# omnirevolve/omnirevolve-image-processor

Hardware: AMD Instinct MI355X
Metric: Mpx/s end-to-end (color->order) (higher is better)
Workload: dtype u8/i32 raster + f32/f64 geometry; 1 GPU; 4096x4096 BGR image, 8 colour layers, stages 02->12 (k-means fit, masks, edges, contours, scale, sort, intra dedup, cross dedup, plot order), default A4 canvas 8400x11880; parallelism=one GPU, one pipeline per colour layer, ops_last_step_rank0=4261, exchange=none

## Files before the change

### omnirevolve-image-processor_amd/csrc/vector08a.hip

```cpp
#include "vec08.h"
#include <rocprim/rocprim.hpp>
#include <type_traits>
#include <vector>

namespace {

template <class Src>
__global__ __launch_bounds__(128) void k_split_small08(Src src, int64_t n_polys, orip_params08 P, const PolyFeat* __restrict__ feat,
                                                        unsigned* __restrict__ is_tap, unsigned* __restrict__ is_keep, int2* __restrict__ tap_xy, GatherDesc* __restrict__ kd) {
    int64_t i = (int64_t)blockIdx.x * blockDim.x + threadIdx.x;
    if (i > n_polys) return;
    if (i == n_polys) { is_tap[i] = 0; is_keep[i] = 0; return; }
    const int64_t n = src.len(i);
    unsigned tap = 0, keep = 0;
    GatherDesc g; g.begin = src.off[i]; g.len = n; g.rev = 0; g.src = (int32_t)i;
    if (n >= 2) {
        const int32_t x0 = feat[i].x0, x1 = feat[i].x1, y0 = feat[i].y0, y1 = feat[i].y1;
        double d = (double)max(x1 - x0, y1 - y0);
        if (d <= P.tap_diam && d <= P.tap_max_dim && n <= (int64_t)P.tap_max_v) {
            double per; float cx, cy, r;
            if constexpr (std::is_same<Src, ESrc>::value) {
                const int32_t* p = reinterpret_cast<const int32_t*>(src.pts + src.off[i]);
                per = (double)vs::pairwise_seglen_sum<0>(p, n);
                if (per <= P.tap_max_per) vs::min_enclosing_circle(p, n, cx, cy, r);
// ... 272 lines not shown
    unsigned i = ord[r]; RsInfo ri = info[i];
    int64_t k = 0;
    if (!ri.pass) k = sample_seg(cum + off[i], ri.n_eff, (double)sample_t(g - sbase[r], step), -1, ri.n_eff - 2);
    hints[b] = make_int2((int)r, (int)k);
}
__device__ __forceinline__ unsigned smp_slot8(unsigned s) { return s ^ ((s >> 5) & 3u); }
__device__ __forceinline__ unsigned smp_slot4(unsigned s) { return s ^ ((s >> 6) & 3u); }
template <int CTRL, int ROWMASK>
__device__ __forceinline__ void wave_seg_step(double& a, unsigned& f) {
    const int lo = __builtin_amdgcn_update_dpp(0, __double2loint(a), CTRL, ROWMASK, 0xf, false);
    const int hi = __builtin_amdgcn_update_dpp(0, __double2hiint(a), CTRL, ROWMASK, 0xf, false);
    const unsigned pf = (unsigned)__builtin_amdgcn_update_dpp(0, (int)f, CTRL, ROWMASK, 0xf, false);
    if (!f) a = __dadd_rn(__hiloint2double(hi, lo), a);
    f |= pf;
}
template <class Src>
__global__ __launch_bounds__(256) void k_samples(Src src, const int64_t* __restrict__ cumoff, const float* __restrict__ cum,
                                                  const RsInfo* __restrict__ info, const unsigned* __restrict__ ord, const unsigned* __restrict__ sbase, int64_t n_rank,
                                                  unsigned MS, double step, int W, int H, SampleArrs A,
                                                  const int2* __restrict__ hints, unsigned nhb, unsigned long long* __restrict__ pixbits, int Wq, unsigned* __restrict__ firstseq) {
    constexpr int S = 4;
    constexpr unsigned NS = 256 * S;
    static_assert(NS == ORIP_SMP_BLOCK, "k_tail_par takes a block of k_samples for 1024 samples");
    __shared__ double shx[NS], shy[NS], shp[2], swa[4];
    __shared__ unsigned swf[4];
    __shared__ unsigned shr[NS];
    const unsigned g0 = (blockIdx.x * 256 + threadIdx.x) * S;
    if (g0 < MS) {
        const unsigned hb = g0 >> 8;
        const int2 h0 = hints[hb];
        const bool last = hb + 1 == nhb;
        const int2 h1 = last ? make_int2((int)n_rank - 1, 0) : hints[hb + 1];
        int64_t r = sample_rank(sbase, info, ord, h0.x + 1, (int64_t)h1.x + 1, g0);
        unsigned i = ord[r]; unsigned j = g0 - sbase[r];
        auto cu = src.cur(i); const float* s = cum + cumoff[i];
        RsInfo ri = info[i];
        int64_t kprev = -2;
        const unsigned j0 = j;
        auto pos_at = [&](int64_t k, double t, double& ox, double& oy) {
            double sk = (double)s[k], sk1 = (double)s[k + 1];
            double u = __ddiv_rn(__dsub_rn(t, sk), fmax(1e-6, __dsub_rn(sk1, sk)));
            double a = __dsub_rn(1.0, u);
            const int2 p0 = cu.at(k), p1 = cu.at(k + 1);
            ox = __dadd_rn(__dmul_rn((double)(float)p0.x, a), __dmul_rn((double)(float)p1.x, u));
            oy = __dadd_rn(__dmul_rn((double)(float)p0.y, a), __dmul_rn((double)(float)p1.y, u));
        };
#pragma unroll 1
        for (int u = 0; u < S; u++) {
            const unsigned g = g0 + (unsigned)u;
            if (g >= MS) break;
            if (u > 0 && j >= ri.m) {
                do { r++; i = ord[r]; ri = info[i]; } while (ri.m == 0);
                j = 0; cu = src.cur(i); s = cum + cumoff[i]; kprev = -2;
            }
            double x, y;
            if (ri.pass) { const int2 q = cu.at(j); x = (double)(float)q.x; y = (double)(float)q.y; }
            else {
                const double t = (double)sample_t(j, step);
                int64_t k;
                if (kprev < -1) {
                    const bool first = u == 0;
                    k = sample_seg(s, ri.n_eff, t, (first && r == h0.x) ? h0.y : -1, (first && !last && r == h1.x) ? h1.y : ri.n_eff - 2);
                } else {
                    k = kprev < 0 ? 0 : kprev;
                    const int64_t kmax = ri.n_eff - 2;
                    while (k < kmax) {
                        float v[8];
#pragma unroll
                        for (int q = 0; q < 8; q++) v[q] = (k + 1 + q <= kmax + 1) ? s[k + 1 + q] : __int_as_float(0x7f800000);
                        int cnt = 0; bool run = true;
#pragma unroll
                        for (int q = 0; q < 8; q++) { run = run && ((double)v[q] <= t); cnt += run ? 1 : 0; }
                        k += cnt;
                        if (cnt < 8) break;
                    }
                    if (k > kmax) k = kmax;
                }
                kprev = k;
                pos_at(k, t, x, y);
            }
            const unsigned ls = threadIdx.x * S + (unsigned)u;
            shx[smp_slot8(ls)] = x; shy[smp_slot8(ls)] = y;
            shr[smp_slot4(ls)] = (unsigned)r | (j == 0 ? 0x80000000u : 0u);
            j++;
        }
        if (j0 > 0 && threadIdx.x == 0) {
            int64_t r2 = sample_rank(sbase, info, ord, h0.x + 1, (int64_t)h1.x + 1, g0);
            const unsigned i2 = ord[r2]; cu = src.cur(i2); s = cum + cumoff[i2]; ri = info[i2];
            double qx, qy;
            if (ri.pass) { const int2 q = cu.at(j0 - 1); qx = (double)(float)q.x; qy = (double)(float)q.y; }
            else { const double t = (double)sample_t(j0 - 1, step); pos_at(sample_seg(s, ri.n_eff, t, -1, ri.n_eff - 2), t, qx, qy); }
            shp[0] = qx; shp[1] = qy;
        }
    }
    __syncthreads();
    const unsigned b0 = blockIdx.x * NS;
    double dd[S] = {0.0, 0.0, 0.0, 0.0};
#pragma unroll
    for (int u = 0; u < S; u++) {
        const unsigned ls = threadIdx.x + 256u * (unsigned)u, g = b0 + ls;
        if (g >= MS) break;
        const unsigned at = smp_slot8(ls);
        const double x = shx[at], y = shy[at];
        const unsigned rw = shr[smp_slot4(ls)];
        double d = 0.0;
        if (!(rw >> 31)) { const unsigned before = smp_slot8(ls ? ls - 1u : 0u); d = vs::norm2_f64(x - (ls ? shx[before] : shp[0]), y - (ls ? shy[before] : shp[1])); }
        A.dprev[g] = d; dd[u] = d;
        A.sx[g] = x; A.sy[g] = y; A.rank[g] = rw & 0x7fffffffu;
        const long long xi = vs::round_half_even(x), yi = vs::round_half_even(y);
        const bool in = xi >= 0 && yi >= 0 && xi < W && yi < H;
        A.pxy[g] = in ? ((unsigned)xi | ((unsigned)yi << 16) | ((rw >> 31) ? ORIP_PXY_FIRST : 0u)) : ORIP_PXY_OUT;
        if (pixbits && in) {
            unsigned long long* wp = &pixbits[(size_t)yi * Wq + (xi >> 6)]; const unsigned long long bit = 1ULL << (xi & 63);
            if (!(*wp & bit) && !(atomicOr(wp, bit) & bit)) firstseq[(size_t)yi * W + xi] = 0xffffffffu;
        }
    }
    __syncthreads();
#pragma unroll
    for (int u = 0; u < S; u++) shx[smp_slot8(threadIdx.x + 256u * (unsigned)u)] = dd[u];
    __syncthreads();
    const unsigned l0 = threadIdx.x * S;
    double v[S]; unsigned f[S];
#pragma unroll
    for (int q = 0; q < S; q++) { v[q] = shx[smp_slot8(l0 + q)]; f[q] = (b0 + l0 + q < MS) ? shr[smp_slot4(l0 + q)] >> 31 : 0u; }
    double wa = v[0]; unsigned wf = f[0];
#pragma unroll
    for (int q = 1; q < S; q++) { wa = f[q] ? v[q] : __dadd_rn(wa, v[q]); wf |= f[q]; }
    wave_seg_step<0x111, 0xf>(wa, wf); wave_seg_step<0x112, 0xf>(wa, wf); wave_seg_step<0x114, 0xf>(wa, wf); wave_seg_step<0x118, 0xf>(wa, wf);
    wave_seg_step<0x142, 0xa>(wa, wf); wave_seg_step<0x143, 0xc>(wa, wf);
    const int lane = threadIdx.x & 63, wv = threadIdx.x >> 6;
    if (lane == 63) { swa[wv] = wa; swf[wv] = wf; }
    double ea = __hiloint2double(__builtin_amdgcn_update_dpp(0, __double2hiint(wa), 0x138 , 0xf, 0xf, false),
                                 __builtin_amdgcn_update_dpp(0, __double2loint(wa), 0x138, 0xf, 0xf, false));
    const unsigned ef = (unsigned)__builtin_amdgcn_update_dpp(0, (int)wf, 0x138, 0xf, 0xf, false);
    __syncthreads();
    if (!ef) {
        double ca = 0.0;
        for (int k = 0; k < wv; k++) ca = swf[k] ? swa[k] : __dadd_rn(ca, swa[k]);
        ea = __dadd_rn(ca, ea);
    }
#pragma unroll
    for (int q = 0; q < S; q++) { ea = f[q] ? v[q] : __dadd_rn(ea, v[q]); v[q] = ea; }
    const unsigned gs = b0 + l0;
    if (gs + S <= MS) { double2* o = reinterpret_cast<double2*>(A.Sloc + gs); o[0] = make_double2(v[0], v[1]); o[1] = make_double2(v[2], v[3]); }
    else { for (int q = 0; q < S; q++) if (gs + q < MS) A.Sloc[gs + q] = v[q]; }
}

__device__ __forceinline__ double dpp_shr1_f64(double v) {
    const int lo = __builtin_amdgcn_update_dpp(0, __double2loint(v), 0x138 , 0xf, 0xf, true);
    const int hi = __builtin_amdgcn_update_dpp(0, __double2hiint(v), 0x138, 0xf, 0xf, true);
    return __hiloint2double(hi, lo);
}
__global__ __launch_bounds__(64) void k_tail_replay(const unsigned* __restrict__ sbase, int64_t n_rank, double T, SampleArrs A, unsigned* __restrict__ npop, const unsigned* __restrict__ only) {
    constexpr unsigned C = 1024u, RM = 2u * C - 1u;
    __shared__ double ops[64], rr[64];
    __shared__ double Dl[2 * C];
    __shared__ unsigned NPl[C];
    const int lane = threadIdx.x;
    for (int64_t r = blockIdx.x; r < n_rank; r += gridDim.x) {
        if (only && !only[r]) continue;
        const unsigned b = sbase[r], e = sbase[r + 1];
        if (e <= b) continue;
        const double* D = A.dprev + b; unsigned* NP = npop + b;
        const unsigned m = e - b;
        unsigned head = 0; double racc = 0.0;
        unsigned j0 = 0, cb = 0;
        auto fill = [&](unsigned c0) {
            double td[16]; unsigned tn[16];
#pragma unroll
            for (int u = 0; u < 16; u++) { const unsigned idx = c0 + (unsigned)lane + 64u * u; td[u] = D[idx < m ? idx : m - 1u]; tn[u] = NP[idx < m ? idx : m - 1u]; }
#pragma unroll
            for (int u = 0; u < 16; u++) { const unsigned idx = c0 + (unsigned)lane + 64u * u; Dl[idx & RM] = td[u]; NPl[idx & (C - 1u)] = tn[u]; }
        };
        auto dist = [&](unsigned idx) -> double { return (idx + C >= cb && idx < cb + C) ? Dl[idx & RM] : D[idx]; };
        auto plain = [&](unsigned s) {
            if (s > head) racc = __dadd_rn(racc, dist(s));
            while (head <= s && racc > T) { head++; if (head <= s) racc = __dsub_rn(racc, dist(head)); else racc = 0.0; }
            if (lane == 0) NP[s] = head;
        };
        fill(0);
        __syncthreads();
        while (j0 < m) {
            if (j0 >= cb + C) { __syncthreads(); cb += C; fill(cb); __syncthreads(); }
            const unsigned s = j0 + (unsigned)lane; const bool valid = s < m && s < cb + C;
            unsigned hp = valid ? NPl[s & (C - 1u)] : 0u;
            hp = hp > head ? hp : head;
            hp = wave_incl_scan_max_u32(hp);
            unsigned prevh = (unsigned)__builtin_amdgcn_update_dpp(0, (int)hp, 0x138 , 0xf, 0xf, true); if (lane == 0) prevh = head;
            const unsigned np = hp - prevh;
            const unsigned inc = valid ? 1u + np : 0u;
            unsigned off = wave_incl_scan_u32(inc);
            const unsigned long long fitm = __ballot(valid && off <= 64u);
            const int m_fit = __popcll(fitm);
            if (m_fit == 0) { plain(j0); j0++; continue; }
            const unsigned total = (unsigned)__builtin_amdgcn_readlane((int)off, m_fit - 1);
            off -= inc;
            if (lane < m_fit) {
                ops[off] = s > prevh ? dist(s) : 0.0;
                for (unsigned t = 0; t < np; t++) ops[off + 1u + t] = -dist(prevh + 1u + t);
            }
            __syncthreads();
            const double v = (unsigned)lane < total ? ops[lane] : 0.0;
            double d = lane == 0 ? __dadd_rn(racc, v) : v;
            double pre = d;
#pragma unroll
            for (int q = 1; q < 64; q++) pre = __dadd_rn(dpp_shr1_f64(pre), d);
            rr[lane] = pre;
            __syncthreads();
            bool bad = false;
            if (lane < m_fit) {
                const double after = rr[off + np];
                bad = after > T || (np > 0u && !(rr[off + np - 1u] > T)) || hp > s;
            }
            const unsigned long long badm = __ballot(bad);
            const int ncommit = badm ? __ffsll((long long)badm) - 1 : m_fit;
            if (lane < ncommit) NP[s] = hp;
            if (ncommit > 0) {
                head = (unsigned)__builtin_amdgcn_readlane((int)hp, ncommit - 1);
                const unsigned last_op = (unsigned)__builtin_amdgcn_readlane((int)(off + np), ncommit - 1);
                racc = rr[last_op];
            }
            __syncthreads();
            j0 += (unsigned)ncommit;
            if (badm) { plain(j0); j0++; }
        }
        __syncthreads();
    }
}

#define ORIP_TAIL_EPS 1e-6
#define ORIP_TAIL_BLOCKS 32u
__global__ __launch_bounds__(256) void k_tail_par(const unsigned* __restrict__ sbase, const unsigned* __restrict__ rank, const double* __restrict__ Sloc, unsigned MS, double T,
                                                   unsigned* __restrict__ npop, unsigned* __restrict__ redo) {
    __shared__ double win[512];
    const unsigned g0 = blockIdx.x * 256, w0 = g0 >= 256 ? g0 - 256 : 0;
    const unsigned KB = g0 / ORIP_SMP_BLOCK, B0 = KB * ORIP_SMP_BLOCK;
    const double lastprev = w0 < B0 ? Sloc[B0 - 1] : 0.0;
    for (unsigned t = threadIdx.x; t < 512; t += 256) {
        const unsigned idx = w0 + t;
        win[t] = (idx < MS && idx < g0 + 256) ? (idx < B0 ? Sloc[idx] - lastprev : Sloc[idx]) : 0.0;
    }
    __syncthreads();
    unsigned g = g0 + threadIdx.x;
    if (g >= MS) return;
    const unsigned r = rank[g], b = sbase[r];
    const double Sj = Sloc[g];
    bool unsure = !(Sj + (b < B0 ? lastprev : 0.0) < 4194304.0) || (g - b) >= (1u << 20);
    unsigned kc = KB; double acc = 0.0;
    auto tail = [&](unsigned p) -> double {
        if (p >= w0) return Sj - win[p - w0];
        const unsigned kb = p / ORIP_SMP_BLOCK;
        if (KB - kb > ORIP_TAIL_BLOCKS) { unsure = true; return __longlong_as_double(0x7ff0000000000000LL); }
        if (kb > kc) { kc = KB; acc = 0.0; }
        while (kc > kb) { kc--; acc += Sloc[kc * ORIP_SMP_BLOCK + (ORIP_SMP_BLOCK - 1u)]; }
        const double up = Sj + acc;
        if (!(up < 4194304.0)) unsure = true;
        return up - Sloc[p];
    };
    unsigned lo = b, hi = g;
    const unsigned wlo = max(b, w0);
    if (wlo == b || !(tail(wlo) <= T)) {
        if (wlo > b) lo = wlo + 1;
        else if (tail(b) <= T) hi = b;
        while (lo < hi) { const unsigned mid = (lo + hi) >> 1; if (tail(mid) <= T) hi = mid; else lo = mid + 1; }
    } else {
        hi = wlo;
        for (unsigned stepb = 1; hi > b; stepb <<= 1) {
            const unsigned p = (hi - b > stepb) ? hi - stepb : b;
            if (tail(p) <= T) { hi = p; if (p == b) break; } else { lo = p + 1; break; }
        }
        while (lo < hi) { const unsigned mid = (lo + hi) >> 1; if (tail(mid) <= T) hi = mid; else lo = mid + 1; }
    }
    const unsigned h = lo;
    if (!(tail(h) <= T - ORIP_TAIL_EPS)) unsure = true;
    if (h > b && !(tail(h - 1) > T + ORIP_TAIL_EPS)) unsure = true;
    npop[g] = h - b;
    if (unsure) redo[r] = 1u;
}
struct IncIndex {
    const unsigned* pxy;
    __device__ unsigned operator()(unsigned g) const { return pxy[g] != ORIP_PXY_OUT ? g + 1u : 0u; }
};
__global__ __launch_bounds__(256) void k_capprev(const unsigned* __restrict__ sbase, unsigned MS, SampleArrs A, const unsigned* __restrict__ lastin, int* __restrict__ capprev) {
    unsigned g = blockIdx.x * 256 + threadIdx.x;
    if (g >= MS) return;
    if (A.pxy[g] == ORIP_PXY_OUT) { capprev[g] = -2; return; }
    const unsigned b = sbase[A.rank[g]];
    const unsigned l = g > b ? lastin[g - 1] : 0u;
    capprev[g] = l ? (int)(l - 1u - b) : -1;
}

__device__ __forceinline__ unsigned long long cap_key(int x0, int y0, int x1, int y1) {
    unsigned long long a = ((unsigned long long)(unsigned)x0 << 14) | (unsigned)y0, b = ((unsigned long long)(unsigned)x1 << 14) | (unsigned)y1;
    if (b < a) { unsigned long long t = a; a = b; b = t; }
    return ((a << 28) | b) + 1ULL;
}
__device__ __forceinline__ unsigned long long hash64(unsigned long long x) { x ^= x >> 33; x *= 0xff51afd7ed558ccdULL; x ^= x >> 33; x *= 0xc4ceb9fe1a85ec53ULL; x ^= x >> 33; return x; }
struct __attribute__((aligned(16))) CapSlot { unsigned long long key; unsigned val; unsigned pad; };
__global__ __launch_bounds__(256) void k_caps_init(CapSlot* __restrict__ tab, unsigned long long tsize, LaneFlags* __restrict__ fl) {
    unsigned long long i = (unsigned long long)blockIdx.x * 256 + threadIdx.x;
    if (i == 0) { fl->caps_overflow = 0; fl->caps_distinct = 0u; fl->accept_survivors = 0u; fl->accept_work = 0ull; }
    if (i < tsize) reinterpret_cast<uint4*>(tab)[i] = make_uint4(0u, 0u, 0xffffffffu, 0u);
}
template <bool CP>
__global__ __launch_bounds__(256) void k_caps_insert(SampleArrs A, const unsigned* __restrict__ sbase, const int* __restrict__ capprev, unsigned MS,
                                                      CapSlot* tab, unsigned long long tmask, int max_probe, int* __restrict__ overflow) {
    constexpr int S = 4;
    const unsigned g0 = blockIdx.x * (256 * S) + threadIdx.x;
    unsigned g[S]; bool on[S];
    unsigned long long key[S], h[S]; unsigned pa[S], pb[S];
#pragma unroll
    for (int u = 0; u < S; u++) { g[u] = g0 + 256u * u; on[u] = g[u] < MS; key[u] = 0; h[u] = 0; pa[u] = 0; pb[u] = 0; }
    if constexpr (CP) {
        unsigned bb[S]; int cp[S];
#pragma unroll
        for (int u = 0; u < S; u++) bb[u] = on[u] ? A.rank[g[u]] : 0u;
#pragma unroll
        for (int u = 0; u < S; u++) if (on[u]) bb[u] = sbase[bb[u]];
#pragma unroll
        for (int u = 0; u < S; u++) { cp[u] = on[u] ? capprev[g[u]] : -1; on[u] = cp[u] >= 0; }
#pragma unroll
        for (int u = 0; u < S; u++) if (on[u]) pa[u] = A.pxy[bb[u] + cp[u]], pb[u] = A.pxy[g[u]];
    } else {
#pragma unroll
        for (int u = 0; u < S; u++) if (on[u]) { pb[u] = A.pxy[g[u]]; pa[u] = g[u] ? A.pxy[g[u] - 1u] : 0u; }
#pragma unroll
        for (int u = 0; u < S; u++) on[u] = on[u] && !(pb[u] & ORIP_PXY_FIRST);
    }
#pragma unroll
    for (int u = 0; u < S; u++) {
        if (on[u]) { key[u] = cap_key(pxy_x(pa[u]), pxy_y(pa[u]), pxy_x(pb[u]), pxy_y(pb[u])); h[u] = hash64(key[u]) & tmask; }
    }
    uint4 sl[S];
#pragma unroll
    for (int u = 0; u < S; u++) sl[u] = on[u] ? *reinterpret_cast<const uint4*>(&tab[h[u]]) : make_uint4(0, 0, 0, 0);
#pragma unroll
    for (int u = 0; u < S; u++) {
        if (!on[u]) continue;
        uint4 s = sl[u]; unsigned long long hh = h[u];
        for (int probe = 0;; probe++) {
            if (probe >= max_probe) { *overflow = 1; break; }
            if (probe) s = *reinterpret_cast<const uint4*>(&tab[hh]);
            unsigned long long cur = ((unsigned long long)s.y << 32) | s.x;
            if (cur == 0) { unsigned long long old = atomicCAS(&tab[hh].key, 0ULL, key[u]); if (old == 0 || old == key[u]) cur = key[u]; else cur = old; }
            if (cur == key[u]) { if (s.z > g[u]) atomicMin(&tab[hh].val, g[u]); break; }
            hh = (hh + 1) & tmask;
        }
    }
}

__global__ __launch_bounds__(256) void k_caps_stamp_bits(const CapSlot* __restrict__ tab, unsigned long long tsize, int rad, unsigned* __restrict__ firstseq, int W, int H,
                                                          const unsigned long long* __restrict__ pixbits, int Wq, unsigned* __restrict__ n_distinct) {
    const int lane = threadIdx.x & 63;
    const long long r2 = (long long)rad * rad;
    unsigned long long wave = ((unsigned long long)blockIdx.x * 256 + threadIdx.x) >> 6, nwaves = ((unsigned long long)gridDim.x * 256) >> 6;
    unsigned mine = 0;
    for (unsigned long long s0 = wave * 64; s0 < tsize; s0 += nwaves * 64) {
        const uint4 sl = (s0 + lane < tsize) ? reinterpret_cast<const uint4*>(tab)[s0 + lane] : make_uint4(0u, 0u, 0u, 0u);
        unsigned long long k = ((unsigned long long)sl.y << 32) | sl.x;
        unsigned v = sl.z;
        unsigned long long occ = __ballot(k != 0);
        mine += (unsigned)__popcll(occ);
        while (occ) {
            int src = __ffsll((long long)occ) - 1; occ &= occ - 1;
            unsigned long long kk = __shfl(k, src, 64) - 1ULL; unsigned seq = __shfl(v, src, 64);
            unsigned long long a = kk >> 28, b = kk & ((1ULL << 28) - 1);
            int x0 = (int)(a >> 14), y0 = (int)(a & 16383), x1 = (int)(b >> 14), y1 = (int)(b & 16383);
            int bx0 = max(0, min(x0, x1) - rad), bx1 = min(W - 1, max(x0, x1) + rad), by0 = max(0, min(y0, y1) - rad), by1 = min(H - 1, max(y0, y1) + rad);
            const int w0 = bx0 >> 6, nw = (bx1 >> 6) - w0 + 1, bh = by1 - by0 + 1;
            for (int i = lane; i < nw * bh; i += 64) {
                const int y = by0 + i / nw, wq = w0 + i % nw;
                unsigned long long bits = pixbits[(size_t)y * Wq + wq];
                const int xb = wq << 6;
                if (xb < bx0) bits &= ~0ULL << (bx0 - xb);
                if (xb + 63 > bx1) bits &= ~0ULL >> (xb + 63 - bx1);
                while (bits) {
                    const int j = __ffsll((long long)bits) - 1; bits &= bits - 1;
                    const int x = xb + j;
                    if (vs::in_capsule(x, y, x0, y0, x1, y1, r2)) { unsigned* q = &firstseq[(size_t)y * W + x]; if (*q > seq) atomicMin(q, seq); }
                }
            }
        }
    }
    if (lane == 0 && mine) atomicAdd(n_distinct, mine);
}

__device__ __forceinline__ unsigned cell_key(long long cx, long long cy) {
    return ((unsigned)((cx + 32768) & 0xffff) << 16) | (unsigned)((cy + 32768) & 0xffff);
}
__global__ __launch_bounds__(256) void k_cell_keys(SampleArrs A, unsigned MS, double inv, unsigned* __restrict__ keys, unsigned* __restrict__ vals) {
    unsigned g = blockIdx.x * 256 + threadIdx.x;
    if (g >= MS) return;
    long long cx = (long long)floor(__dmul_rn(A.sx[g], inv)), cy = (long long)floor(__dmul_rn(A.sy[g], inv));
    keys[g] = cell_key(cx, cy); vals[g] = g;
}
__global__ __launch_bounds__(256) void k_accept_pre(SampleArrs A, const unsigned* __restrict__ sbase, const unsigned* __restrict__ npop, unsigned MS,
                                                     const unsigned* __restrict__ firstseq, int W, uint8_t* __restrict__ sflag,
                                                     unsigned* __restrict__ surv, unsigned* __restrict__ n_surv, unsigned long long* __restrict__ work) {
    constexpr int S = 4;
    const unsigned g0 = blockIdx.x * (256 * S) + threadIdx.x;
    unsigned g[S], bb[S], np[S]; int xi[S], yi[S]; bool ok[S], on[S];
#pragma unroll
    for (int u = 0; u < S; u++) { g[u] = g0 + 256u * u; on[u] = g[u] < MS; bb[u] = on[u] ? A.rank[g[u]] : 0u; }
#pragma unroll
    for (int u = 0; u < S; u++) {
        np[u] = 0; xi[u] = 0; yi[u] = 0; ok[u] = false;
        if (on[u]) { bb[u] = sbase[bb[u]]; const unsigned p = A.pxy[g[u]]; ok[u] = p != ORIP_PXY_OUT; np[u] = npop[g[u]]; xi[u] = pxy_x(p); yi[u] = pxy_y(p); }
    }
    unsigned fs[S];
#pragma unroll
    for (int u = 0; u < S; u++) fs[u] = (on[u] && ok[u]) ? firstseq[(size_t)yi[u] * W + xi[u]] : 0xffffffffu;
    const int lane = threadIdx.x & 63;
#pragma unroll
    for (int u = 0; u < S; u++) {
        bool need = false; unsigned mynp = 0;
        if (on[u]) {
            const unsigned j = g[u] - bb[u];
            const unsigned limit = bb[u] + np[u];
            bool k = ok[u];
            if (k && fs[u] < limit) k = false;
            sflag[g[u]] = (k ? 1 : 0) | (j == 0 ? 2 : 0);
            need = k && np[u] > 0; mynp = need ? np[u] : 0u;
        }
        const unsigned long long m = __ballot(need);
        if (m) {
            unsigned long long wsum = mynp;
            for (int o = 32; o > 0; o >>= 1) wsum += __shfl_xor(wsum, o, 64);
            unsigned base = 0;
            if (lane == 0) { base = atomicAdd(n_surv, (unsigned)__popcll(m)); atomicAdd(work, wsum); }
            base = (unsigned)__shfl((int)base, 0, 64);
            if (need) surv[base + (unsigned)__popcll(m & ((1ull << lane) - 1ull))] = g[u];
        }
    }
}
__global__ __launch_bounds__(256) void k_accept_brute(SampleArrs A, const unsigned* __restrict__ sbase, const unsigned* __restrict__ npop, double R2,
                                                       const unsigned* __restrict__ surv, const unsigned* __restrict__ n_surv, uint8_t* __restrict__ sflag) {
    const unsigned ns = *n_surv;
    const int lane = threadIdx.x & 63;
    for (unsigned t = blockIdx.x * 4 + (threadIdx.x >> 6); t < ns; t += gridDim.x * 4) {
        const unsigned g = surv[t];
        const unsigned b = sbase[A.rank[g]], np = npop[g];
        const double x = A.sx[g], y = A.sy[g];
        bool rej = false;
        for (unsigned q0 = 0; q0 < np && !rej; q0 += 64) {
            const unsigned q = q0 + (unsigned)lane; bool hit = false;
            if (q < np) {
                double ddx = __dsub_rn(A.sx[b + q], x), ddy = __dsub_rn(A.sy[b + q], y);
                hit = __dadd_rn(__dmul_rn(ddx, ddx), __dmul_rn(ddy, ddy)) <= R2;
            }
            if (__ballot(hit)) rej = true;
        }
        if (rej && lane == 0) sflag[g] &= (uint8_t)~1u;
    }
}
__global__ __launch_bounds__(256) void k_accept(SampleArrs A, const unsigned* __restrict__ sbase, const unsigned* __restrict__ npop, double inv, double R2,
                                                 const unsigned* __restrict__ skeys, const unsigned* __restrict__ svals,
                                                 const unsigned* __restrict__ surv, const unsigned* __restrict__ n_surv, uint8_t* __restrict__ sflag) {
    const unsigned ns = *n_surv;
    const int lane = threadIdx.x & 63;
    for (unsigned t = blockIdx.x * 4 + (threadIdx.x >> 6); t < ns; t += gridDim.x * 4) {
        const unsigned g = surv[t];
        const unsigned r = A.rank[g], b = sbase[r];
        const double x = A.sx[g], y = A.sy[g];
        const unsigned limit = b + npop[g];
        const long long cx = (long long)floor(__dmul_rn(x, inv)), cy = (long long)floor(__dmul_rn(y, inv));
        const long long seg_end = sbase[r + 1];
        bool rej = false;
        for (int dx = -1; dx <= 1 && !rej; dx++) {
            const unsigned key_lo = cell_key(cx + dx, cy - 1), key_hi = cell_key(cx + dx, cy + 1);
            long long lo = b, hi = seg_end;
            while (hi - lo > 0) {
                const long long w = (hi - lo + 64) / 65;
                const long long pos = lo + (long long)(lane + 1) * w - 1;
                const bool below = pos < hi && skeys[pos] < key_lo;
                const int cnt = __popcll(__ballot(below));
                const long long nlo = lo + (long long)cnt * w;
                const long long nhi = (cnt < 64) ? min(hi, lo + (long long)(cnt + 1) * w - 1) : hi;
                lo = min(nlo, hi); hi = nhi;
            }
            for (long long q = lo; q < seg_end; q += 64) {
                const long long idx = q + lane;
                bool in = false, hit = false;
                if (idx < seg_end) {
                    const unsigned k = skeys[idx];
                    in = k <= key_hi;
                    if (in) {
                        const unsigned g2 = svals[idx];
                        if (g2 < limit) {
                            double ddx = __dsub_rn(A.sx[g2], x), ddy = __dsub_rn(A.sy[g2], y);
                            hit = __dadd_rn(__dmul_rn(ddx, ddx), __dmul_rn(ddy, ddy)) <= R2;
                        }
                    }
                }
                if (__ballot(hit)) { rej = true; break; }
                if (__ballot(in) != ~0ull) break;
            }
        }
        if (rej && lane == 0) sflag[g] &= (uint8_t)~1u;
    }
}

__global__ __launch_bounds__(256) void k_pf_views(const PolyFeat* __restrict__ feat07, const int64_t* __restrict__ off, int64_t n, VView* __restrict__ vf, VView* __restrict__ vr,
                                                   int64_t* __restrict__ lf, int64_t* __restrict__ lr) {
    int64_t i = (int64_t)blockIdx.x * 256 + threadIdx.x;
    if (i == n) { lf[i] = 0; lr[i] = 0; }
    if (i >= n) return;
    const unsigned len = (unsigned)(off[i + 1] - off[i]);
    VView a; a.wid = (unsigned)i; a.first = 0u; a.len = (feat07[i].closed && len > 0u) ? len - 1u : len; a.rev = 0u;
    VView b; b.wid = (unsigned)i; b.first = 0u; b.len = len; b.rev = 1u;
    vf[i] = a; vr[i] = b; lf[i] = a.len; lr[i] = b.len;
}
__global__ __launch_bounds__(256) void k_pf_pick_feat(const VView* __restrict__ sview, int64_t n, const PolyFeat* __restrict__ pf, const float* __restrict__ per_rev, PolyFeat* __restrict__ out) {
    int64_t k = (int64_t)blockIdx.x * 256 + threadIdx.x;
    if (k >= n) return;
    const VView v = sview[k];
    PolyFeat f = pf[v.wid];
    if (v.rev) { const int32_t ax = f.sx, ay = f.sy; f.sx = f.ex; f.sy = f.ey; f.ex = ax; f.ey = ay; f.per = per_rev[v.wid]; }
    out[k] = f;
}
__global__ __launch_bounds__(256) void k_pf_pick_info(const VView* __restrict__ kview, int64_t nk, const RsInfo* __restrict__ pinfo, int64_t npf, const int64_t* __restrict__ off_f,
                                                       const int64_t* __restrict__ off_r, int64_t tot_f, RsInfo* __restrict__ info, int64_t* __restrict__ cumoff) {
    int64_t j = (int64_t)blockIdx.x * 256 + threadIdx.x;
    if (j >= nk) return;
    const VView v = kview[j];
    info[j] = pinfo[v.rev ? npf + (int64_t)v.wid : (int64_t)v.wid];
    cumoff[j] = v.rev ? tot_f + off_r[v.wid] : off_f[v.wid];
}
struct StreamSwap {
    LaneRes& l;
    explicit StreamSwap(LaneRes& lane) : l(lane) { std::swap(l.stream, l.stream2); }
    ~StreamSwap() { std::swap(l.stream, l.stream2); }
};
static std::atomic<uint64_t> g_pf_tag{1};
}
int orip_prefetch08(orip_ctx* c, const orip_params08& P, DPolys& S, const PolyFeat* feat07) {
    LaneRes::Prefetch08& F = LN(c).pf08;
    F.valid = false;
    const int64_t n = S.n, total = S.total;
    if (n <= 0 || total <= 0 || total > 0x3fffffff) return 0;
    const double step = std::max(1.0, P.sample_step);
    HIPC(c, F.feat.ensure((size_t)n * (sizeof(PolyFeat) + 4) + 64));
    HIPC(c, F.info.ensure((size_t)2 * n * sizeof(RsInfo) + 64));
    HIPC(c, F.cum.ensure((size_t)2 * total * 4 + 64));
    HIPC(c, F.ord.ensure((size_t)n * 16 + 64));
    HIPC(c, F.seg.ensure((size_t)total * 4 + 64));
    {
        StreamSwap sw(LN(c));
        HIPC(c, hipStreamWaitEvent(LN(c).stream, LN(c).ev2, 0));
        PolyFeat* ff = F.feat.as<PolyFeat>(); float* per_rev = reinterpret_cast<float*>(ff + n); RsInfo* inf = F.info.as<RsInfo>(); float* cum = F.cum.as<float>();
        VSrc sS; ORIP_TRY(vsrc_of(c, S, sS));
        vfeatures_short(c, sS, n, VF_PER | VF_OPEN_VIEW | VF_PER_REV, ff, per_rev);
        unsigned* kin = F.ord.as<unsigned>(); unsigned* kout = kin + n; unsigned* vin = kout + n; unsigned* ordl = vin + n;
        float* seg = F.seg.as<float>();
        ORIP_TRY(vlen_order(c, S.off.as<int64_t>(), n, kin, kout, vin, ordl));
        HIPC(c, hipEventRecord(LN(c).ev4, LN(c).stream));
        HIPC(c, hipStreamWaitEvent(LN(c).stream2 , LN(c).ev4, 0));
        if (total > ORIP_LONG_CUM) {
            { ProfScope ps(c, "k_seglen"); hipLaunchKernelGGL(k_seglen<VSrc>, dim3((unsigned)cdiv(total, 4 * 63 * 64)), dim3(256), 0, LN(c).stream, sS, n, total, seg, ff); }
            if (total > ORIP_LONG_POLY) ORIP_TRY(vfeatures_long_seg(c, sS, n, total, ff, ordl, per_rev, seg));
        }
        HIPC(c, hipEventRecord(LN(c).ev4, LN(c).stream));
        { ProfScope ps(c, "k_cumlen"); hipLaunchKernelGGL(k_cumlen2<VSrc>, dim3(cdiv(2 * n, 128)), dim3(128), 0, LN(c).stream, sS, feat07, n, step, cum, total, inf); }
        if (total > ORIP_LONG_CUM) { ProfScope ps(c, "k_cumlen_long"); const dim3 grid((unsigned)std::min<int64_t>(n, 8192), 2);
            hipLaunchKernelGGL(k_cumlen_long2<VSrc>, grid, dim3(64), 0, LN(c).stream, sS, n, step, cum, total, inf, ordl, 0, (const float*)seg); }
        HIPC(c, hipGetLastError());
        HIPC(c, hipEventRecord(LN(c).ev3, LN(c).stream));
    }
    F.pending = true;
    F.valid = true; F.tag = g_pf_tag.fetch_add(1); F.n = n; F.tot_f = total; F.step = step; F.src_off = S.off.as<int64_t>();
    return 0;
}
namespace {

int split_small(orip_ctx* c, DPolys& src, const orip_params08& P, DPolys& kept, DBuf& tapbuf, int64_t tap_base, int64_t* n_taps_out, PolyFeat* kept_feat = nullptr) {
    *n_taps_out = 0;
    HIPC(c, kept.clear(LN(c).stream));
    int64_t n = src.n;
    if (n == 0) return 0;
    unsigned *is_tap, *is_keep, *tap_scan, *keep_scan; int2* tap_xy; GatherDesc *kd, *kd2;
    { Carve L; L.each(n + 1, is_tap, is_keep, tap_scan, keep_scan, tap_xy, kd, kd2); HIPC(c, L.commit(LN(c).vtmp[VTL_SPLIT], 256)); }
    HIPC(c, LN(c).vtmp[VTL_SPLIT_FEAT].ensure((size_t)n * sizeof(PolyFeat) + 64));
    PolyFeat* sfeat = LN(c).vtmp[VTL_SPLIT_FEAT].as<PolyFeat>();
    if (is_coded(src) && P.tap_max_v > 64) ORIP_TRY(orip_polys_materialize(c, src));
    LaneRes::Prefetch08& F = LN(c).pf08;
    if (kept_feat && is_coded(src) && src.pf_tag && F.valid && F.tag == src.pf_tag && !src.vident) {
        if (F.pending) HIPC(c, hipStreamWaitEvent(LN(c).stream, LN(c).ev4, 0));
        hipLaunchKernelGGL(k_pf_pick_feat, dim3(cdiv(n, 256)), dim3(256), 0, LN(c).stream, src.vview.as<VView>(), n, F.feat.as<PolyFeat>(), reinterpret_cast<const float*>(F.feat.as<PolyFeat>() + F.n), sfeat);
    } else { HIPC(c, orip_pf08_drain(c)); ORIP_TRY(vfeatures(c, src, kept_feat ? (VF_PER | VF_OPEN_VIEW) : 0, sfeat)); }
    { ProfScope ps(c, "k_split_small08"); ORIP_WITH_SRC(c, src, sv, { hipLaunchKernelGGL(k_split_small08<decltype(sv)>, dim3(cdiv(n + 1, 128)), dim3(128), 0, LN(c).stream, sv, n, P, sfeat, is_tap, is_keep, tap_xy, kd); }); }
    ORIP_TRY(vscan_excl<unsigned>(c, is_tap, tap_scan, (size_t)n + 1));
    ORIP_TRY(vscan_excl<unsigned>(c, is_keep, keep_scan, (size_t)n + 1));
    unsigned nt = 0, nk = 0;
    HIPC(c, hipMemcpyAsync(&nt, tap_scan + n, 4, hipMemcpyDeviceToHost, LN(c).stream));
    ORIP_TRY(vread(c, &nk, keep_scan + n));
    if (nt) {
        HIPC(c, tapbuf.ensure((size_t)(tap_base + nt) * 8 + 64, LN(c).stream, true));
        hipLaunchKernelGGL(k_compact<int2>, dim3(cdiv(n, 256)), dim3(256), 0, LN(c).stream, is_tap, tap_scan, n, tap_xy, tapbuf.as<int2>() + tap_base);
    }
    *n_taps_out = nt;
    if (nk) {
        hipLaunchKernelGGL(k_compact<GatherDesc>, dim3(cdiv(n, 256)), dim3(256), 0, LN(c).stream, is_keep, keep_scan, n, kd, kd2);
        ORIP_TRY(vgather_list(c, kd2, nk, src, kept));
        if (kept_feat) hipLaunchKernelGGL(k_compact<PolyFeat>, dim3(cdiv(n, 256)), dim3(256), 0, LN(c).stream, is_keep, keep_scan, n, sfeat, kept_feat);
    }
    HIPC(c, hipGetLastError());
    return 0;
}

__global__ __launch_bounds__(256) void k_fill_per(const PolyFeat* __restrict__ f, int64_t n, float* __restrict__ k, unsigned* __restrict__ v, unsigned* __restrict__ any_out) {
    int64_t i = (int64_t)blockIdx.x * 256 + threadIdx.x;
    if (i == 0) *any_out = 0u;
    if (i < n) { k[i] = f[i].per; v[i] = (unsigned)i; }
}

struct A08 {
    int64_t nk;
    PolyFeat* feat;
    unsigned *ord, *mr, *sbase; RsInfo* info;
    unsigned* redo;
    double step; int64_t* cumoff; float* cum;
    unsigned MS; bool any_out;
    SampleArrs A; unsigned* npop; int* capprev; uint8_t* sflag;
    unsigned *ckin, *ckout, *cvin, *cvout; int2* hints;
    double cell, inv;
    int Wq; unsigned* firstseq; unsigned long long* pixbits;
};

static int a1_order(orip_ctx* c, A08& a) {
    const int64_t nk = a.nk; float *kin, *kout; unsigned* vin;
    { Carve L; L.each(nk, kin, kout, vin, a.ord); L.take(a.mr, nk + 1);
      L.take(a.sbase, nk + 2); L.take(a.info, nk); L.take(a.redo, nk + 1); HIPC(c, L.commit(LN(c).vtmp[VTL_RANKS], 256)); }
    hipLaunchKernelGGL(k_fill_per, dim3(cdiv(nk, 256)), dim3(256), 0, LN(c).stream, a.feat, nk, kin, vin, a.sbase + nk + 1);
    ORIP_TRY((vsort_pairs<float, unsigned>(c, kin, kout, vin, a.ord, (size_t)nk, 0, 32, true)));
    return 0;
}
static int a2_resample(orip_ctx* c, const orip_params08& P, DPolys& kept0, A08& a, PhaseTimer& T) {
    const int W = P.W, H = P.H; const int64_t nk = a.nk;
    a.step = std::max(1.0, P.sample_step);
    const LaneRes::Prefetch08& F = LN(c).pf08;
    const bool picked = is_coded(kept0) && kept0.pf_tag && F.valid && F.tag == kept0.pf_tag && F.step == a.step && !kept0.vident;
    HIPC(c, orip_pf08_drain(c));
    { Carve L; L.take(a.cumoff, nk + 1); L.take(a.cum, picked ? 0 : kept0.total); HIPC(c, L.commit(LN(c).vtmp[VTL_CUM], 128)); }
    if (picked) {
        a.cum = F.cum.as<float>();
        hipLaunchKernelGGL(k_pf_pick_info, dim3(cdiv(nk, 256)), dim3(256), 0, LN(c).stream, kept0.vview.as<VView>(), nk, F.info.as<RsInfo>(), F.n, F.src_off, F.src_off, F.tot_f, a.info, a.cumoff);
    } else {
        HIPC(c, hipMemcpyAsync(a.cumoff, kept0.off.p, (size_t)(nk + 1) * 8, hipMemcpyDeviceToDevice, LN(c).stream));
        { ProfScope ps(c, "k_cumlen"); ORIP_WITH_SRC(c, kept0, sv, { hipLaunchKernelGGL(k_cumlen<decltype(sv)>, dim3(cdiv(nk, 128)), dim3(128), 0, LN(c).stream, sv, nk, a.step, a.cum, a.info); }); }
        if (kept0.total > ORIP_LONG_CUM) { ProfScope ps(c, "k_cumlen_long"); ORIP_WITH_SRC(c, kept0, sv, {
                hipLaunchKernelGGL(k_cumlen_long2<decltype(sv)>, dim3((unsigned)std::min<int64_t>(nk, 8192), 1), dim3(64), 0, LN(c).stream, sv, nk, a.step, a.cum, (int64_t)0, a.info, a.ord, 0, (const float*)nullptr); }); }
    }
    T.tick("cumlen");
    hipLaunchKernelGGL(k_rank_counts, dim3(cdiv(nk + 1, 256)), dim3(256), 0, LN(c).stream, a.info, a.ord, nk, a.mr, a.feat, W, H, a.sbase + nk + 1, a.redo);
    ORIP_TRY(vscan_excl<unsigned>(c, a.mr, a.sbase, (size_t)nk + 1));
    unsigned ms_out[2] = {0, 0};
    ORIP_TRY(vread(c, ms_out, a.sbase + nk, 2));
    const unsigned MS = a.MS = ms_out[0]; a.any_out = ms_out[1] != 0 || getenv("ORIP_CAPPREV_SCAN");
    if (MS == 0) return 0;
    if (MS > 0x7ffffff0u) ORIP_FAIL(c, "too many samples");
    if (T.on) { char b[48]; snprintf(b, sizeof b, " [MS %u]", MS); T.log += b; }
    { Carve L; L.each(MS, a.A.sx, a.A.sy, a.A.dprev, a.A.pxy, a.A.rank, a.npop, a.capprev, a.sflag); HIPC(c, L.commit(LN(c).vtmp[VTL_SAMPLES], 1024)); }
    { Carve L; L.take(a.A.Sloc, MS); HIPC(c, L.commit(LN(c).vtmp[VTL_TAIL_RUNS], 64)); }
    const unsigned nb = (unsigned)cdiv(MS, 256);
    { Carve L; L.each(MS, a.ckin, a.ckout, a.cvin, a.cvout); L.take(a.hints, nb + 1, 64);
      HIPC(c, L.commit(LN(c).vtmp[VTL_CELLS], 64 + (size_t)MS * 8)); }
    a.cell = P.grid_stride > 0 ? P.grid_stride : std::max(4.0, P.col_rad); a.inv = 1.0 / a.cell;
    a.Wq = (W + 63) >> 6;
    HIPC(c, LN(c).canvas.ensure((size_t)W * H * 4 + 64));
    a.firstseq = LN(c).canvas.as<unsigned>();
    HIPC(c, LN(c).pixbits.ensure((size_t)a.Wq * H * 8 + 64));
    a.pixbits = LN(c).pixbits.as<unsigned long long>();
    HIPC(c, hipMemsetAsync(a.pixbits, 0, (size_t)a.Wq * H * 8, LN(c).stream));
    hipLaunchKernelGGL(k_sample_hints, dim3(cdiv(nb, 256)), dim3(256), 0, LN(c).stream, a.cumoff, a.cum, a.info, a.ord, a.sbase, nk, MS, a.step, nb, a.hints);
    { ProfScope ps(c, "k_samples"); ORIP_WITH_SRC(c, kept0, sv, { hipLaunchKernelGGL(k_samples<decltype(sv)>, dim3(cdiv(nb, 4)), dim3(256), 0, LN(c).stream, sv, a.cumoff, a.cum, a.info, a.ord, a.sbase, nk, MS, a.step, W, H, a.A, a.hints, (unsigned)nb, a.pixbits, a.Wq, a.firstseq); }); }
    T.tick("samples");
    return 0;
}
static void tail_dbg_dump(orip_ctx* c, int layer, const A08& a) {
    const int64_t nk = a.nk;
    std::vector<unsigned> h(nk), sb(nk + 1);
    hipStreamSynchronize(LN(c).stream);
    hipMemcpy(h.data(), a.redo, nk * 4, hipMemcpyDeviceToHost);
    hipMemcpy(sb.data(), a.sbase, (nk + 1) * 4, hipMemcpyDeviceToHost);
    unsigned long long nf = 0, sf = 0, mx = 0;
    for (int64_t q = 0; q < nk; q++) if (h[q]) { nf++; sf += sb[q + 1] - sb[q]; mx = std::max<unsigned long long>(mx, sb[q + 1] - sb[q]); }
    fprintf(stderr, "[tail dbg] layer %d: %llu of %lld polylines redone, %llu of %u samples, longest redone %llu\n", layer, nf, (long long)nk, sf, a.MS, mx);
}
static int a3_tails(orip_ctx* c, int layer, const orip_params08& P, A08& a) {
    const int64_t nk = a.nk; const unsigned MS = a.MS;
    {
        ProfScope ps(c, "k_tail_sim");
        hipLaunchKernelGGL(k_tail_par, dim3(cdiv(MS, 256)), dim3(256), 0, LN(c).stream, a.sbase, a.A.rank, a.A.Sloc, MS, P.tail_len_px, a.npop, a.redo);
        if (getenv("ORIP_TAIL_DBG")) tail_dbg_dump(c, layer, a);
        const unsigned* only = getenv("ORIP_TAIL_SEQ") ? nullptr : a.redo;
        HIPC(c, hipEventRecord(LN(c).ev2, LN(c).stream));
        HIPC(c, hipStreamWaitEvent(LN(c).stream2, LN(c).ev2, 0));
        hipLaunchKernelGGL(k_tail_replay, dim3((unsigned)std::min<int64_t>(nk, 65535)), dim3(64), 0, LN(c).stream2, a.sbase, nk, P.tail_len_px, a.A, a.npop, only);
        HIPC(c, hipEventRecord(LN(c).ev3, LN(c).stream2));
    }
    if (a.any_out) {
        unsigned* lastin = LN(c).vtmp[VTL_TAIL_RUNS].as<unsigned>();
        auto vin = rocprim::make_transform_iterator(rocprim::counting_iterator<unsigned>(0u), IncIndex{a.A.pxy});
        HIPC(c, orip_with_tmp(c, [&](void* tmp, size_t& bytes) { return rocprim::inclusive_scan_by_key(tmp, bytes, a.A.rank, vin, lastin, (size_t)MS, rocprim::maximum<unsigned>(), rocprim::equal_to<unsigned>(), LN(c).stream); }));
        hipLaunchKernelGGL(k_capprev, dim3(cdiv(MS, 256)), dim3(256), 0, LN(c).stream, a.sbase, MS, a.A, lastin, a.capprev);
    }
    else a.capprev = nullptr;
    return 0;
}
static int a4_capsules(orip_ctx* c, const orip_params08& P, A08& a) {
    const unsigned MS = a.MS; LaneFlags* fl = LN(c).flags.as<LaneFlags>();
    unsigned long long tfull = 1024; while (tfull < 2ull * MS) tfull <<= 1;
    unsigned long long tsize = 1024;
    if (LN(c).caps_hint) { while (tsize < 3ull * LN(c).caps_hint) tsize <<= 1; } else { while (tsize < MS / 4ull) tsize <<= 1; }
    tsize = std::min(tsize, tfull);
    if (getenv("ORIP_CAPS_TINY")) tsize = 1024;
    CapSlot* tab = nullptr;
    int* d_ovf = &fl->caps_overflow; unsigned* d_dist = &fl->caps_distinct;
    for (;; tsize = std::min(tfull, tsize * 4)) {
        HIPC(c, LN(c).vtmp[VTL_CAPS].ensure((size_t)tsize * 16 + 64));
        tab = LN(c).vtmp[VTL_CAPS].as<CapSlot>();
        hipLaunchKernelGGL(k_caps_init, dim3((unsigned)cdiv(tsize, 256)), dim3(256), 0, LN(c).stream, tab, tsize, fl);
        const int max_probe = tsize >= tfull ? 0x7fffffff : 96;
        { ProfScope ps(c, "k_caps_insert");
          if (a.capprev) hipLaunchKernelGGL(k_caps_insert<true>, dim3(cdiv(MS, 1024)), dim3(256), 0, LN(c).stream, a.A, a.sbase, a.capprev, MS, tab, tsize - 1, max_probe, d_ovf);
          else hipLaunchKernelGGL(k_caps_insert<false>, dim3(cdiv(MS, 1024)), dim3(256), 0, LN(c).stream, a.A, a.sbase, a.capprev, MS, tab, tsize - 1, max_probe, d_ovf); }
        int ovf = 0; ORIP_TRY(vread(c, &ovf, d_ovf));
        if (!ovf) break;
    }
    {
        ProfScope ps(c, "k_caps_stamp");
        const dim3 sg((unsigned)std::min<unsigned long long>(tsize / 64 / 4 + 1, 16384));
        hipLaunchKernelGGL(k_caps_stamp_bits, sg, dim3(256), 0, LN(c).stream, tab, tsize, P.brush_forbid / 2, a.firstseq, P.W, P.H, a.pixbits, a.Wq, d_dist);
    }
    return 0;
}
static int a56_accept(orip_ctx* c, const orip_params08& P, A08& a, PhaseTimer& T) {
    const int64_t nk = a.nk; const unsigned MS = a.MS; LaneFlags* fl = LN(c).flags.as<LaneFlags>();
    HIPC(c, hipStreamWaitEvent(LN(c).stream, LN(c).ev3, 0));
    unsigned* surv = LN(c).vtmp[VTL_TAIL_RUNS].as<unsigned>();
    unsigned* d_ns = &fl->accept_survivors; unsigned long long* d_work = &fl->accept_work;
    { ProfScope ps(c, "k_accept"); hipLaunchKernelGGL(k_accept_pre, dim3(cdiv(MS, 1024)), dim3(256), 0, LN(c).stream, a.A, a.sbase, a.npop, MS, a.firstseq, P.W, a.sflag, surv, d_ns, d_work); }
    unsigned long long h_work = 0; ORIP_TRY(vread(c, &h_work, d_work));
    const double R2 = P.col_rad * P.col_rad;
    const bool brute = a.cell >= P.col_rad && h_work <= 64ull * (unsigned long long)MS && !getenv("ORIP_HASH_SORT");
    if (T.on) { char b2[64]; snprintf(b2, sizeof b2, " [near work %llu %s]", h_work, brute ? "direct" : "buckets"); T.log += b2; }
    if (brute) {
        ProfScope ps(c, "k_accept");
        hipLaunchKernelGGL(k_accept_brute, dim3((unsigned)std::min<unsigned>(cdiv(MS, 256), 16384u)), dim3(256), 0, LN(c).stream, a.A, a.sbase, a.npop, R2, surv, d_ns, a.sflag);
    } else {
        hipLaunchKernelGGL(k_cell_keys, dim3(cdiv(MS, 256)), dim3(256), 0, LN(c).stream, a.A, MS, a.inv, a.ckin, a.cvin);
        { ProfScope ps(c, "sort_cells"); HIPC(c, orip_with_tmp(c, [&](void* tmp, size_t& bytes) { return rocprim::segmented_radix_sort_pairs(tmp, bytes, a.ckin, a.ckout, a.cvin, a.cvout, (unsigned)MS, (unsigned)nk, a.sbase, a.sbase + 1, 0u, 32u, LN(c).stream); })); }
        ProfScope ps(c, "k_accept");
        hipLaunchKernelGGL(k_accept, dim3((unsigned)std::min<unsigned>(cdiv(MS, 256), 16384u)), dim3(256), 0, LN(c).stream, a.A, a.sbase, a.npop, a.inv, R2, a.ckout, a.cvout, surv, d_ns, a.sflag);
    }
    HIPC(c, hipGetLastError());
    return 0;
}
}

int dedup08_a(orip_ctx* c, int layer, const orip_params08& P, DPolys& S, DTaps& TOUT, PhaseTimer& T, bool& caps_counted) {
    DPolys& kept0 = LN(c).tp[0]; DPolys& cleaned = LN(c).tp[1]; DPolys& lines2 = LN(c).tp[2];
    int64_t nt0 = 0, nt2 = 0;
    A08 a{};
    HIPC(c, LN(c).vtmp[VTL_FEAT].ensure((size_t)S.n * sizeof(PolyFeat) + 64));
    a.feat = LN(c).vtmp[VTL_FEAT].as<PolyFeat>();
    ORIP_TRY(split_small(c, S, P, kept0, TOUT.xy, 0, &nt0, a.feat));
    a.nk = kept0.n;
    T.tick("split");
    if (a.nk > 0) {
        if (kept0.total > 0x7fffffff) ORIP_FAIL(c, "layer too large");
        T.tick("feat");
        ORIP_TRY(a1_order(c, a));                          T.tick("A0-1");
        ORIP_TRY(a2_resample(c, P, kept0, a, T));
        if (a.MS > 0) {
            ORIP_TRY(a3_tails(c, layer, P, a));            T.tick("tail");
            ORIP_TRY(a4_capsules(c, P, a));                caps_counted = true; T.tick("caps");
            ORIP_TRY(a56_accept(c, P, a, T));              T.tick("accept");
            ORIP_TRY(orip_runs_to_polys(c, SlotPtsF64{a.A.sx, a.A.sy}, a.sflag, a.MS, cleaned));
            T.tick("runs");
        }
        ORIP_TRY(split_small(c, cleaned, P, lines2, TOUT.xy, nt0, &nt2));
    }
    TOUT.n = nt0 + nt2;
    return 0;
}
```

Baseline: 254.8 Mpx/s.

## Pre-deduplicate capsule keys in an LDS hash set before global table insertion

The capsule insert kernel now gives each block a range of several 1024-sample chunks. Each block deduplicates capsule keys in a small shared-memory hash set with bounded probing, and only the per-block minimum-index owner of each key goes on to the global hash table. Loads for the next chunk are software-prefetched while the current chunk is hashed. The aim is fewer global atomics and less table traffic when many samples share capsules. In exchange it adds shared-memory atomics, a __syncthreads per chunk, and fewer blocks in flight. An env override picks the range and set size.

After: 283.8 Mpx/s (median of 6 runs). 11.4% higher.

```diff
diff --git a/omnirevolve-image-processor_amd/csrc/vector08a.hip b/omnirevolve-image-processor_amd/csrc/vector08a.hip
--- a/omnirevolve-image-processor_amd/csrc/vector08a.hip
+++ b/omnirevolve-image-processor_amd/csrc/vector08a.hip
@@ -598,49 +598,79 @@
     if (i == 0) { fl->caps_overflow = 0; fl->caps_distinct = 0u; fl->accept_survivors = 0u; fl->accept_work = 0ull; }
     if (i < tsize) reinterpret_cast<uint4*>(tab)[i] = make_uint4(0u, 0u, 0xffffffffu, 0u);
 }
+constexpr int ORIP_CAPSSET_PROBES = 4;
+constexpr int ORIP_CAPSSET_SHIFT = 52;
 template <bool CP>
 __global__ __launch_bounds__(256) void k_caps_insert(SampleArrs A, const unsigned* __restrict__ sbase, const int* __restrict__ capprev, unsigned MS,
+                                                      unsigned chunks, unsigned smask,
                                                       CapSlot* tab, unsigned long long tmask, int max_probe, int* __restrict__ overflow) {
     constexpr int S = 4;
-    const unsigned g0 = blockIdx.x * (256 * S) + threadIdx.x;
-    unsigned g[S]; bool on[S];
-    unsigned long long key[S], h[S]; unsigned pa[S], pb[S];
-#pragma unroll
-    for (int u = 0; u < S; u++) { g[u] = g0 + 256u * u; on[u] = g[u] < MS; key[u] = 0; h[u] = 0; pa[u] = 0; pb[u] = 0; }
-    if constexpr (CP) {
-        unsigned bb[S]; int cp[S];
-#pragma unroll
-        for (int u = 0; u < S; u++) bb[u] = on[u] ? A.rank[g[u]] : 0u;
-#pragma unroll
-        for (int u = 0; u < S; u++) if (on[u]) bb[u] = sbase[bb[u]];
-#pragma unroll
-        for (int u = 0; u < S; u++) { cp[u] = on[u] ? capprev[g[u]] : -1; on[u] = cp[u] >= 0; }
-#pragma unroll
-        for (int u = 0; u < S; u++) if (on[u]) pa[u] = A.pxy[bb[u] + cp[u]], pb[u] = A.pxy[g[u]];
-    } else {
-#pragma unroll
-        for (int u = 0; u < S; u++) if (on[u]) { pb[u] = A.pxy[g[u]]; pa[u] = g[u] ? A.pxy[g[u] - 1u] : 0u; }
-#pragma unroll
-        for (int u = 0; u < S; u++) on[u] = on[u] && !(pb[u] & ORIP_PXY_FIRST);
-    }
-#pragma unroll
-    for (int u = 0; u < S; u++) {
-        if (on[u]) { key[u] = cap_key(pxy_x(pa[u]), pxy_y(pa[u]), pxy_x(pb[u]), pxy_y(pb[u])); h[u] = hash64(key[u]) & tmask; }
-    }
-    uint4 sl[S];
-#pragma unroll
-    for (int u = 0; u < S; u++) sl[u] = on[u] ? *reinterpret_cast<const uint4*>(&tab[h[u]]) : make_uint4(0, 0, 0, 0);
-#pragma unroll
-    for (int u = 0; u < S; u++) {
-        if (!on[u]) continue;
-        uint4 s = sl[u]; unsigned long long hh = h[u];
-        for (int probe = 0;; probe++) {
-            if (probe >= max_probe) { *overflow = 1; break; }
-            if (probe) s = *reinterpret_cast<const uint4*>(&tab[hh]);
-            unsigned long long cur = ((unsigned long long)s.y << 32) | s.x;
-            if (cur == 0) { unsigned long long old = atomicCAS(&tab[hh].key, 0ULL, key[u]); if (old == 0 || old == key[u]) cur = key[u]; else cur = old; }
-            if (cur == key[u]) { if (s.z > g[u]) atomicMin(&tab[hh].val, g[u]); break; }
-            hh = (hh + 1) & tmask;
+    extern __shared__ unsigned long long caps_set[];
+    unsigned long long* skey = caps_set; unsigned* sval = reinterpret_cast<unsigned*>(caps_set + (smask + 1u));
+    for (unsigned i = threadIdx.x; i <= smask; i += 256) { skey[i] = 0ULL; sval[i] = 0xffffffffu; }
+    __syncthreads();
+    const unsigned long long first = (unsigned long long)blockIdx.x * chunks * 1024ull;
+    const unsigned long long left = (unsigned long long)MS - first;
+    const unsigned nch = left < chunks * 1024ull ? (unsigned)((left + 1023ull) >> 10) : chunks;
+    auto pixels = [&](unsigned ch, unsigned (&pa)[S], unsigned (&pb)[S], bool (&on)[S]) {
+        unsigned g[S];
+#pragma unroll
+        for (int u = 0; u < S; u++) { g[u] = (unsigned)first + ch * 1024u + threadIdx.x + 256u * u; on[u] = ch < nch && g[u] < MS; pa[u] = 0; pb[u] = 0; }
+        if constexpr (CP) {
+            unsigned bb[S]; int cp[S];
+#pragma unroll
+            for (int u = 0; u < S; u++) bb[u] = on[u] ? A.rank[g[u]] : 0u;
+#pragma unroll
+            for (int u = 0; u < S; u++) if (on[u]) bb[u] = sbase[bb[u]];
+#pragma unroll
+            for (int u = 0; u < S; u++) { cp[u] = on[u] ? capprev[g[u]] : -1; on[u] = cp[u] >= 0; }
+#pragma unroll
+            for (int u = 0; u < S; u++) if (on[u]) pa[u] = A.pxy[bb[u] + cp[u]], pb[u] = A.pxy[g[u]];
+        } else {
+#pragma unroll
+            for (int u = 0; u < S; u++) if (on[u]) { pb[u] = A.pxy[g[u]]; pa[u] = g[u] ? A.pxy[g[u] - 1u] : 0u; }
+        }
+    };
+    unsigned npa[S], npb[S]; bool non[S];
+    pixels(0, npa, npb, non);
+    for (unsigned ch = 0; ch < nch; ch++) {
+        unsigned g[S]; bool on[S]; unsigned long long key[S], h[S]; int ss[S];
+#pragma unroll
+        for (int u = 0; u < S; u++) {
+            g[u] = (unsigned)first + ch * 1024u + threadIdx.x + 256u * u; key[u] = 0; h[u] = 0; ss[u] = -1;
+            on[u] = non[u]; if constexpr (!CP) on[u] = on[u] && !(npb[u] & ORIP_PXY_FIRST);
+            if (on[u]) key[u] = cap_key(pxy_x(npa[u]), pxy_y(npa[u]), pxy_x(npb[u]), pxy_y(npb[u]));
+        }
+        pixels(ch + 1, npa, npb, non);
+#pragma unroll
+        for (int u = 0; u < S; u++) {
+            if (!on[u]) continue;
+            const unsigned long long hs = hash64(key[u]);
+            h[u] = hs & tmask;
+            unsigned i = (unsigned)(hs >> ORIP_CAPSSET_SHIFT) & smask;
+            for (int p = 0; p < ORIP_CAPSSET_PROBES; p++, i = (i + 1u) & smask) {
+                const unsigned long long old = atomicCAS(&skey[i], 0ULL, key[u]);
+                if (old == 0ULL || old == key[u]) { atomicMin(&sval[i], g[u]); ss[u] = (int)i; break; }
+            }
+        }
+        __syncthreads();
+#pragma unroll
+        for (int u = 0; u < S; u++) on[u] = on[u] && (ss[u] < 0 || sval[ss[u]] == g[u]);
+        uint4 sl[S];
+#pragma unroll
+        for (int u = 0; u < S; u++) sl[u] = on[u] ? *reinterpret_cast<const uint4*>(&tab[h[u]]) : make_uint4(0, 0, 0, 0);
+#pragma unroll
+        for (int u = 0; u < S; u++) {
+            if (!on[u]) continue;
+            uint4 s = sl[u]; unsigned long long hh = h[u];
+            for (int probe = 0;; probe++) {
+                if (probe >= max_probe) { *overflow = 1; break; }
+                if (probe) s = *reinterpret_cast<const uint4*>(&tab[hh]);
+                unsigned long long cur = ((unsigned long long)s.y << 32) | s.x;
+                if (cur == 0) { unsigned long long old = atomicCAS(&tab[hh].key, 0ULL, key[u]); if (old == 0 || old == key[u]) cur = key[u]; else cur = old; }
+                if (cur == key[u]) { if (s.z > g[u]) atomicMin(&tab[hh].val, g[u]); break; }
+                hh = (hh + 1) & tmask;
+            }
         }
     }
 }
@@ -1010,6 +1040,18 @@
     if (LN(c).caps_hint) { while (tsize < 3ull * LN(c).caps_hint) tsize <<= 1; } else { while (tsize < MS / 4ull) tsize <<= 1; }
     tsize = std::min(tsize, tfull);
     if (getenv("ORIP_CAPS_TINY")) tsize = 1024;
+    static const unsigned cand[] = {8192u, 4096u, 2048u, 1024u};
+    unsigned R = 1024u, TS = 2048u;
+    for (unsigned r : cand) if (cdiv(MS, r) >= 2048 || r == 1024u) { R = r; break; }
+    if (const char* e = getenv("ORIP_CAPS_RANGE")) {
+        char* end = nullptr; const unsigned long r = strtoul(e, &end, 10); unsigned long t = TS;
+        if (end && *end == ':') t = strtoul(end + 1, nullptr, 10);
+        if (r < 1024 || r > 65536 || (r & 1023)) ORIP_FAIL(c, "ORIP_CAPS_RANGE: a multiple of 1024 up to 65536");
+        if (t < 32 || t > 4096 || (t & (t - 1))) ORIP_FAIL(c, "ORIP_CAPS_RANGE: a power of two from 32 to 4096 slots");
+        R = (unsigned)r; TS = (unsigned)t;
+    }
+    if (getenv("ORIP_CAPSSET_TINY")) TS = 32u;
+    const unsigned lds = TS * 12u;
     CapSlot* tab = nullptr;
     int* d_ovf = &fl->caps_overflow; unsigned* d_dist = &fl->caps_distinct;
     for (;; tsize = std::min(tfull, tsize * 4)) {
@@ -1018,8 +1060,8 @@
         hipLaunchKernelGGL(k_caps_init, dim3((unsigned)cdiv(tsize, 256)), dim3(256), 0, LN(c).stream, tab, tsize, fl);
         const int max_probe = tsize >= tfull ? 0x7fffffff : 96;
         { ProfScope ps(c, "k_caps_insert");
-          if (a.capprev) hipLaunchKernelGGL(k_caps_insert<true>, dim3(cdiv(MS, 1024)), dim3(256), 0, LN(c).stream, a.A, a.sbase, a.capprev, MS, tab, tsize - 1, max_probe, d_ovf);
-          else hipLaunchKernelGGL(k_caps_insert<false>, dim3(cdiv(MS, 1024)), dim3(256), 0, LN(c).stream, a.A, a.sbase, a.capprev, MS, tab, tsize - 1, max_probe, d_ovf); }
+          if (a.capprev) hipLaunchKernelGGL(k_caps_insert<true>, dim3(cdiv(MS, R)), dim3(256), lds, LN(c).stream, a.A, a.sbase, a.capprev, MS, R / 1024u, TS - 1u, tab, tsize - 1, max_probe, d_ovf);
+          else hipLaunchKernelGGL(k_caps_insert<false>, dim3(cdiv(MS, R)), dim3(256), lds, LN(c).stream, a.A, a.sbase, a.capprev, MS, R / 1024u, TS - 1u, tab, tsize - 1, max_probe, d_ovf); }
         int ovf = 0; ORIP_TRY(vread(c, &ovf, d_ovf));
         if (!ovf) break;
     }
```
